# abowman6/CBET_RayTracing_3D

Measured on AMD Instinct MI355X. Metric: ray-steps/sec, OMEGA 60-beam 256^3 sweep, higher is better.
Workload: dtype f64

## Files before the change

cbet_raytracing_3d_amd/api.py:

```python
import ctypes as C
import os

import numpy as np

_PKG = os.path.dirname(os.path.abspath(__file__))
LIB_PATH = os.environ.get("CBET_LIB_PATH") or os.path.join(_PKG, "lib", "libcbet_mi355x.so")
DATA_DIR = os.path.join(_PKG, "data")

OK, EINVAL, EHIP, ENOMEM, ENODEVICE, ECOMM = 0, -1, -2, -3, -4, -5
NPHASE = 2001
KERNEL_DEFAULT, KERNEL_GLOBAL_ATOMICS, KERNEL_LDS_COMBINE, KERNEL_LDS_WINDOW = 0, 1, 2, 3


class CbetError(RuntimeError):
    def __init__(self, code, msg):
        super().__init__("cbet error %d: %s" % (code, msg))
        self.code = code


class Params(C.Structure):
    _fields_ = [
        ("nx", C.c_int), ("ny", C.c_int), ("nz", C.c_int),
        ("xmin", C.c_double), ("xmax", C.c_double),
        ("ymin", C.c_double), ("ymax", C.c_double),
# ... 101 lines not shown
    return hist


EXPORTS = [
    "cbet_last_error", "cbet_version", "cbet_params_default", "cbet_derive",
    "cbet_live_ray_list", "cbet_omega60_beam_norm", "cbet_host_power_table", "cbet_host_beam_trig", "cbet_read_profile",
    "cbet_safeGPUAlloc", "cbet_moveToAndFromGPU", "cbet_gpuFree",
    "cbet_context_create", "cbet_context_destroy", "cbet_context_counters", "cbet_context_tables", "cbet_context_set_launch_list",
    "cbet_launch_ray_XYZ", "cbet_tabulate_plasma", "cbet_trace_nodes", "cbet_prepare_step_records", "cbet_ray_tracing",
    "cbet_write_text", "cbet_edep_average", "cbet_edep_average_device", "cbet_node_coordinates", "cbet_write_npy",
    "cbet_debug_bounds_violations",
    "cbet_gain_params_default", "cbet_gain_constants", "cbet_trace_cbet", "cbet_gain_field",
    "cbet_cbet_workspace_bytes", "cbet_cbet_solve", "cbet_gain_field_slab", "cbet_gain_field_packed",
    "cbet_cbet_slab_workspace_bytes", "cbet_cbet_slab_workspace_bytes_parts", "cbet_pack_segments", "cbet_unpack_segments",
    "cbet_context_list_length", "cbet_cbet_workspace_gain", "cbet_trace_exits", "cbet_exit_tally", "cbet_farfield",
    "cbet_sph_modes_device", "cbet_sph_modes", "cbet_prepare_plasma", "cbet_context_step_records",
]

_lib = None


def lib():
    global _lib
    if _lib is not None:
        return _lib
    import torch
    if not os.path.exists(LIB_PATH):
        raise ImportError(
            "%s is missing: build it with `python -m cbet_raytracing_3d_amd.build` "
            "(hipcc --offload-arch=gfx950).  There is no CPU fallback." % LIB_PATH)
    L = C.CDLL(LIB_PATH)
# ... 8 lines not shown
    L.cbet_host_beam_trig.argtypes = [dp, C.c_int, dp]
    L.cbet_read_profile.argtypes = [C.c_char_p, C.c_int, dp, dp]
    L.cbet_safeGPUAlloc.argtypes = [C.POINTER(vp), C.c_size_t, C.c_int]
    L.cbet_moveToAndFromGPU.argtypes = [vp, vp, C.c_size_t, C.c_int]
    L.cbet_gpuFree.argtypes = [vp, C.c_int]
    L.cbet_context_create.argtypes = [C.POINTER(vp), C.POINTER(Params), C.c_int]
    L.cbet_context_destroy.argtypes = [vp]
    L.cbet_context_counters.argtypes = [vp, vp, C.POINTER(Counters), C.c_int]
    L.cbet_context_set_launch_list.argtypes = [vp, ip, C.c_long]
    L.cbet_context_tables.argtypes = [vp, C.POINTER(vp), C.POINTER(vp)]
    L.cbet_launch_ray_XYZ.argtypes = [C.c_int, C.c_uint, vp, vp, vp, vp, vp, vp, vp, vp,
                                      C.c_double, C.c_double, C.c_double, C.POINTER(Params), vp, vp]
    L.cbet_tabulate_plasma.argtypes = [vp, C.POINTER(Params), vp, vp, vp, vp]
    L.cbet_prepare_step_records.argtypes = [vp, C.POINTER(Params), vp, vp, C.c_double, C.c_double, C.c_double, vp]
    L.cbet_prepare_plasma.argtypes = [vp, C.POINTER(Params), vp, vp, vp, C.c_double, C.c_double, C.c_double, vp]
    L.cbet_context_step_records.argtypes = [vp, C.POINTER(vp), C.POINTER(C.c_ulonglong)]
    L.cbet_trace_nodes.argtypes = [C.c_int, C.c_uint, vp, vp, vp, vp, vp, vp, vp,
                                   C.c_double, C.c_double, C.c_double, C.POINTER(Params), vp, vp]
    L.cbet_ray_tracing.argtypes = [dp, dp, dp, dp, C.POINTER(Params), dp, ip, C.c_int, dp,
                                   C.POINTER(Counters)]
    L.cbet_debug_bounds_violations.argtypes = [C.POINTER(C.c_ulonglong), C.c_int, vp]
    L.cbet_write_text.argtypes = [dp, C.c_int, C.c_int, C.c_int, C.c_char_p]
    L.cbet_write_text.restype = C.c_longlong
    L.cbet_edep_average.argtypes = [dp, dp, C.c_int, C.c_int, C.c_int]
    L.cbet_edep_average_device.argtypes = [vp, vp, C.c_int, C.c_int, C.c_int, vp]
    L.cbet_node_coordinates.argtypes = [C.POINTER(Params), dp, dp, dp]
    L.cbet_write_npy.argtypes = [dp, C.c_int, C.POINTER(C.c_long), C.c_char_p]
    L.cbet_write_npy.restype = C.c_longlong
    L.cbet_gain_params_default.argtypes = [C.POINTER(GainParams)]
    L.cbet_gain_constants.argtypes = [C.POINTER(Params), C.POINTER(GainParams), dp, dp, dp]
# ... 197 lines not shown
def tabulate_plasma(ctx, params, te_data_g, r_data_g, ne_data_g, stream=None):
    _check(lib().cbet_tabulate_plasma(ctx.handle, C.byref(params), _addr(te_data_g),
                                      _addr(r_data_g), _addr(ne_data_g), _addr(stream)))


def prepare_step_records(ctx, params, ne3d, kappa3d, xconst, yconst, zconst, stream=None):
    _check(lib().cbet_prepare_step_records(ctx.handle, C.byref(params), _addr(ne3d), _addr(kappa3d), xconst, yconst,
                                           zconst, _addr(stream)))


def prepare_plasma(ctx, params, te_data_g, r_data_g, ne_data_g, xconst, yconst, zconst, stream=None):
    _check(lib().cbet_prepare_plasma(ctx.handle, C.byref(params), _addr(te_data_g), _addr(r_data_g), _addr(ne_data_g),
                                     xconst, yconst, zconst, _addr(stream)))


def trace_nodes(b, nindices, ne3d, kappa3d, edep, bbeam_norm, beam_norm, pow_r, phase_r, xconst,
                yconst, zconst, params, ctx, stream=None):
    _check(lib().cbet_trace_nodes(
        b, nindices, _addr(ne3d), _addr(kappa3d), _addr(edep), _addr(bbeam_norm), _addr(beam_norm),
        _addr(pow_r), _addr(phase_r), xconst, yconst, zconst, C.byref(params), ctx.handle,
        _addr(stream)))


def default_gain_params(**overrides):
    g = GainParams()
    _check(lib().cbet_gain_params_default(C.byref(g)))
    for k, v in overrides.items():
        setattr(g, k, v)
    return g

# ... 180 lines not shown
```

cbet_raytracing_3d_amd/csrc/cbet_abi.cpp:

```cpp
#include <hip/hip_runtime_api.h>

#include <algorithm>
#include <cmath>
#include <cstdarg>
#include <cstdio>
#include <cstdlib>
#include <cstring>
#include <map>
#include <mutex>
#include <vector>

#include "cbet_device.h"
#include "cbet_mi355x.h"
#include "cbet_omega_beams.h"

namespace cbet {

thread_local char g_err[512] = "";

int fail(int code, const char *fmt, ...)
{
    va_list ap;
    va_start(ap, fmt);
    vsnprintf(g_err, sizeof g_err, fmt, ap);
// ... 196 lines not shown

}

using namespace cbet;

struct cbet_context {
    int gpu = -1;
    cbet_params p{};
    cbet_derived d{};
    double *ne3d = nullptr, *kap3d = nullptr;
    StepRecord *steprec = nullptr;
    unsigned long long tables_version = 0, rec_version = ~0ull;
    unsigned long long rec_builds = 0;
    const double *rec_ne3d = nullptr, *rec_kap3d = nullptr;
    double rec_const[3] = {0, 0, 0};
    double *xlaunch = nullptr, *ylaunch = nullptr;
    double *bounds = nullptr;
    int *live = nullptr;
    int nlive = 0;
    unsigned long long *counters = nullptr;
};

extern "C" {

const char *cbet_last_error(void) { return g_err; }
const char *cbet_version(void) { return "cbet-mi355x 0.1 (gfx950, hip)"; }

int cbet_params_default(cbet_params *p, int n)
{
    if (!p) return fail(CBET_EINVAL, "params is NULL");
// ... 260 lines not shown
{
    if (!out) return fail(CBET_EINVAL, "out is NULL");
    hipError_t e = audit_violations(out, reset != 0, (hipStream_t)stream);
    if (e == hipErrorNotSupported) return fail(CBET_EINVAL, "not a bounds-audit build (compile with -DCBET_DEBUG_BOUNDS)");
    if (e != hipSuccess) return fail(CBET_EHIP, "audit_violations: %s", hipGetErrorString(e));
    return CBET_OK;
}

int cbet_context_list_length(const cbet_context *ctx, long *length)
{
    if (!ctx || !length) return fail(CBET_EINVAL, "NULL context/length");
    *length = ctx->nlive;
    return CBET_OK;
}

int cbet_context_tables(cbet_context *ctx, double **ne3d, double **kappa3d)
{
    if (!ctx) return fail(CBET_EINVAL, "NULL context");
    if (ne3d) *ne3d = ctx->ne3d;
    if (kappa3d) *kappa3d = ctx->kap3d;
    ++ctx->tables_version;
    return CBET_OK;
}

int cbet_context_step_records(const cbet_context *ctx, const void **records, unsigned long long *builds)
{
    if (!ctx) return fail(CBET_EINVAL, "NULL context");
    if (records) *records = ctx->steprec;
    if (builds) *builds = ctx->rec_builds;
    return CBET_OK;
}

static int check_geometry(const cbet_context *ctx, const cbet_params *p)
// ... 5 lines not shown
        p->max_threads != q.max_threads || p->threads_per_block != q.threads_per_block ||
        p->courant_mult != q.courant_mult || p->patch_order != q.patch_order || p->rim_merge != q.rim_merge)
        return fail(CBET_EINVAL, "launch parameters do not match the geometry the context was created for");
    return CBET_OK;
}

int cbet_tabulate_plasma(cbet_context *ctx, const cbet_params *p, const double *te_data_g,
                         const double *r_data_g, const double *ne_data_g, void *stream)
{
    if (!ctx) return fail(CBET_EINVAL, "NULL context");
    if (int rc = validate(p)) return rc;
    if (int rc = check_geometry(ctx, p)) return rc;
    if (!te_data_g || !r_data_g || !ne_data_g) return fail(CBET_EINVAL, "NULL profile pointer");
    DeviceGuard guard;
    CBET_HIP(hipSetDevice(ctx->gpu));
    TabulateArgs t{};
    t.nx = p->nx; t.ny = p->ny; t.nz = p->nz; t.nprofile = p->nprofile;
    t.xmin = p->xmin; t.ymin = p->ymin; t.zmin = p->zmin;
    t.dx = ctx->d.dx; t.dy = ctx->d.dy; t.dz = ctx->d.dz; t.dt = ctx->d.dt;
    t.ncrit = ctx->d.ncrit;
    t.r = r_data_g; t.ne = ne_data_g; t.te = te_data_g;
    t.ne3d = ctx->ne3d; t.kap3d = ctx->kap3d;
    CBET_HIP(launch_tabulate(t, (hipStream_t)stream));
    ++ctx->tables_version;
    return CBET_OK;
}

static int step_records(cbet_context *ctx, const cbet_params *p, const double *ne3d, const double *kappa3d,
                        double xconst, double yconst, double zconst, void *stream, bool force)
{
    const bool own = !ne3d && !kappa3d;
    const double *ne = ne3d ? ne3d : ctx->ne3d, *kap = kappa3d ? kappa3d : ctx->kap3d;
    if (!force && own && ctx->rec_version == ctx->tables_version && ctx->rec_ne3d == ne && ctx->rec_kap3d == kap &&
        ctx->rec_const[0] == xconst && ctx->rec_const[1] == yconst && ctx->rec_const[2] == zconst)
        return CBET_OK;
    StepTableArgs t{};
    t.nx = p->nx; t.ny = p->ny; t.nz = p->nz;
    t.xconst = xconst; t.yconst = yconst; t.zconst = zconst;
    t.ne3d = ne; t.kap3d = kap; t.rec = ctx->steprec;
    CBET_HIP(launch_step_table(t, (hipStream_t)stream));
    ++ctx->rec_builds;
    ctx->rec_version = own ? ctx->tables_version : ~0ull;
    ctx->rec_ne3d = ne; ctx->rec_kap3d = kap;
    ctx->rec_const[0] = xconst; ctx->rec_const[1] = yconst; ctx->rec_const[2] = zconst;
    return CBET_OK;
}

int cbet_prepare_step_records(cbet_context *ctx, const cbet_params *p, const double *ne3d, const double *kappa3d,
                              double xconst, double yconst, double zconst, void *stream)
{
    if (!ctx) return fail(CBET_EINVAL, "NULL context");
    if (int rc = validate(p)) return rc;
    if (int rc = check_geometry(ctx, p)) return rc;
    DeviceGuard guard;
    CBET_HIP(hipSetDevice(ctx->gpu));
    return step_records(ctx, p, ne3d, kappa3d, xconst, yconst, zconst, stream, true);
}

int cbet_prepare_plasma(cbet_context *ctx, const cbet_params *p, const double *te_data_g, const double *r_data_g,
                        const double *ne_data_g, double xconst, double yconst, double zconst, void *stream)
{
    if (!ctx) return fail(CBET_EINVAL, "NULL context");
    if (int rc = validate(p)) return rc;
    if (int rc = check_geometry(ctx, p)) return rc;
    if (!te_data_g || !r_data_g || !ne_data_g) return fail(CBET_EINVAL, "NULL profile pointer");
    if (plasma_records_lds(p->nprofile) > 65536) {
        if (int rc = cbet_tabulate_plasma(ctx, p, te_data_g, r_data_g, ne_data_g, stream)) return rc;
        return cbet_prepare_step_records(ctx, p, nullptr, nullptr, xconst, yconst, zconst, stream);
    }
    DeviceGuard guard;
    CBET_HIP(hipSetDevice(ctx->gpu));
    PlasmaRecordsArgs a{};
    TabulateArgs &t = a.t;
    t.nx = p->nx; t.ny = p->ny; t.nz = p->nz; t.nprofile = p->nprofile;
    t.xmin = p->xmin; t.ymin = p->ymin; t.zmin = p->zmin;
    t.dx = ctx->d.dx; t.dy = ctx->d.dy; t.dz = ctx->d.dz; t.dt = ctx->d.dt;
    t.ncrit = ctx->d.ncrit;
    t.r = r_data_g; t.ne = ne_data_g; t.te = te_data_g;
    t.ne3d = ctx->ne3d; t.kap3d = ctx->kap3d;
    a.xconst = xconst; a.yconst = yconst; a.zconst = zconst;
    a.rec = ctx->steprec;
    CBET_HIP(launch_plasma_records(a, (hipStream_t)stream));
    ++ctx->tables_version;
    ++ctx->rec_builds;
    ctx->rec_version = ctx->tables_version;
    ctx->rec_ne3d = ctx->ne3d; ctx->rec_kap3d = ctx->kap3d;
    ctx->rec_const[0] = xconst; ctx->rec_const[1] = yconst; ctx->rec_const[2] = zconst;
    return CBET_OK;
}

struct CbetHooks {
    const double *gain = nullptr;
    int quantity = 0;
    double *beam_gain = nullptr;
    double max_exponent = 0.0;
    bool exits = false;
};

static int trace_impl(int b, unsigned nindices, const double *ne3d, const double *kappa3d,
                      double *edep, const double *bbeam_norm, const double *beam_norm,
                      const double *pow_r, const double *phase_r, double xconst, double yconst,
                      double zconst, const cbet_params *p, cbet_context *ctx, void *stream,
                      const CbetHooks &hooks)
// ... 41 lines not shown
    a.xconst = xconst; a.yconst = yconst; a.zconst = zconst;
    a.nt = d.nt; a.absorption = p->absorption;
    a.rpz = p->rays_per_zone; a.zones = d.zones_spanned; a.nrays_x = d.nrays_x;
    a.z_launch = kFocal - d.dz / 2;
    a.uray_mult = d.uray_mult; a.omega = d.omega; a.ncrit = d.ncrit;
    a.xlaunch = ctx->xlaunch; a.ylaunch = ctx->ylaunch;
    a.live = ctx->live; a.nlive = ctx->nlive;
    a.beam_lo = beam_lo; a.nbeams_local = beam_hi - beam_lo;
    a.bundles_per_beam = (ctx->nlive + kWave - 1) / kWave;
    a.total_bundles = (long)a.nbeams_local * a.bundles_per_beam;
    {
        const long K = p->shard_count > 1 ? p->shard_count : 1, r = p->shard_count > 1 ? p->shard_index : 0;
        a.first_item = (r * a.total_bundles) / K;
        a.item_count = ((r + 1) * a.total_bundles) / K - a.first_item;
    }
    a.ne3d = ne3d ? ne3d : ctx->ne3d;
    a.kap3d = kappa3d ? kappa3d : ctx->kap3d;
    a.beam_norm = beam_norm; a.bbeam_norm = bbeam_norm; a.pow_r = pow_r; a.phase_r = phase_r;
    a.edep = edep;
    a.sYh = p->edep_zpitch > 0 ? p->edep_zpitch : p->nz + 2;
    a.sXh = (p->ny + 2) * a.sYh;
    if (p->edep_zpitch > 0 && (p->per_beam_grids || cbet_hooks))
        return fail(CBET_EINVAL, "edep_zpitch applies to the plain path's single deposit grid (no per-beam grids, no CBET hooks)");
    a.grid_stride = (p->per_beam_grids || hooks.quantity != 0) ? d.edep_size : 0;
    if (hooks.exits) a.grid_stride = (long)kExitDoubles * ctx->nlive;
    const int gb_n = p->grid_beams > 0 ? p->grid_beams : p->nbeams, gb_0 = p->grid_beams > 0 ? p->grid_beam0 : 0;
    if ((a.grid_stride != 0 || hooks.gain) && (beam_lo < gb_0 || beam_hi > gb_0 + gb_n))
        return fail(CBET_EINVAL, "beams [%d,%d) are not all inside the beam-resolved arrays' range [%d,%d)", beam_lo, beam_hi,
                    gb_0, gb_0 + gb_n);
    a.grid_beam0 = gb_0;
    a.comp_stride = (long)gb_n * d.edep_size;
    a.counters = ctx->counters;
    a.stats = p->window_stats != 0;
    a.gain = hooks.gain; a.hsize = d.edep_size; a.quantity = hooks.quantity;
    a.max_exponent = hooks.max_exponent; a.beam_gain = hooks.beam_gain;
    DeviceGuard guard;
    CBET_HIP(hipSetDevice(ctx->gpu));
    if (variant == CBET_KERNEL_LDS_WINDOW) {
        if (int rc = step_records(ctx, p, ne3d, kappa3d, xconst, yconst, zconst, stream, false)) return rc;
        a.steprec = ctx->steprec;
    }
    CBET_HIP(launch_trace(a, hooks.exits ? kTraceExits : variant, p->force_wide_index != 0, (hipStream_t)stream));
    return CBET_OK;
}

int cbet_trace_nodes(int b, unsigned nindices, const double *ne3d, const double *kappa3d,
                     double *edep, const double *bbeam_norm, const double *beam_norm,
                     const double *pow_r, const double *phase_r, double xconst, double yconst,
                     double zconst, const cbet_params *p, cbet_context *ctx, void *stream)
{
    return trace_impl(b, nindices, ne3d, kappa3d, edep, bbeam_norm, beam_norm, pow_r, phase_r, xconst, yconst,
                      zconst, p, ctx, stream, CbetHooks{});
}

static std::mutex g_ctx_mu;
// ... 18 lines not shown
    g_default_ctx[dev] = ctx;
    *out = ctx;
    return CBET_OK;
}

int cbet_launch_ray_XYZ(int b, unsigned nindices, double *te_data_g, double *r_data_g,
                        double *ne_data_g, double *edep, double *bbeam_norm, double *beam_norm,
                        double *pow_r, double *phase_r, double xconst, double yconst,
                        double zconst, const cbet_params *p, cbet_context *ctx, void *stream)
{
    if (int rc = validate(p)) return rc;
    if (!ctx) {
        if (int rc = default_context(p, &ctx)) return rc;
    }
    const bool records = p->kernel_variant == CBET_KERNEL_DEFAULT || p->kernel_variant == CBET_KERNEL_LDS_WINDOW;
    if (int rc = records ? cbet_prepare_plasma(ctx, p, te_data_g, r_data_g, ne_data_g, xconst, yconst, zconst, stream)
                         : cbet_tabulate_plasma(ctx, p, te_data_g, r_data_g, ne_data_g, stream)) return rc;
    return cbet_trace_nodes(b, nindices, nullptr, nullptr, edep, bbeam_norm, beam_norm, pow_r, phase_r,
                            xconst, yconst, zconst, p, ctx, stream);
}

int cbet_edep_average_device(const double *edep, double *edepavg, int nx, int ny, int nz, void *stream)
{
    if (!edep || !edepavg || nx < 1 || ny < 1 || nz < 1) return fail(CBET_EINVAL, "cbet_edep_average_device: bad array");
    if ((long)(nx + 2) * (ny + 2) * (nz + 2) >= (1L << 31)) return fail(CBET_EINVAL, "cbet_edep_average_device: grid too large");
    CBET_HIP(launch_edep_average(edep, edepavg, nx, ny, nz, (hipStream_t)stream));
    return CBET_OK;
}

int cbet_pack_segments(const double *src, long beam_stride, int hy, int hz, const int *segments, long nseg, double *out,
                       void *stream)
// ... 142 lines not shown
    a.dx = d.dx; a.dy = d.dy; a.dz = d.dz; a.dt = d.dt;
    a.ncrit = d.ncrit; a.k0 = d.omega / kC;
    a.cs = cs; a.gain_const = gc; a.iaw = g->iaw;
    a.mach_r0 = g->mach_r0; a.mach_0 = g->mach_0; a.mach_r1 = g->mach_r1; a.mach_1 = g->mach_1;
    a.relax = g->relax;
    a.fields = fields; a.ne3d = ne3d ? ne3d : ctx->ne3d; a.gain = gain; a.scratch = scratch; a.change = change;
    a.hx_lo = hx_lo; a.hx_hi = hx_hi;
    a.consume = (consume && scratch) ? 1 : 0;
    a.frozen = g->directions_frozen ? 1 : 0;
    const long plane = (long)(p->ny + 2) * (p->nz + 2);
    a.store0 = packed ? (long)hx_lo * plane : 0;
    a.bstride = packed ? (long)(hx_hi - hx_lo) * plane : d.edep_size;
    if (hx_hi == hx_lo) return CBET_OK;
    DeviceGuard guard;
    CBET_HIP(hipSetDevice(ctx->gpu));
    CBET_HIP(launch_gain_field(a, (hipStream_t)stream));
    return CBET_OK;
}

size_t cbet_cbet_workspace_bytes(const cbet_params *p)
{
    if (!p || validate(p) != CBET_OK) return 0;
    const size_t hsize = (size_t)(p->nx + 2) * (p->ny + 2) * (p->nz + 2);
    return (5 * (size_t)p->nbeams * hsize + 2 + CBET_MAX_CBET_BEAMS) * sizeof(double);
}

int cbet_cbet_solve(double *te_data_g, double *r_data_g, double *ne_data_g, double *edep,
                    double *bbeam_norm, double *beam_norm, double *pow_r, double *phase_r,
                    const cbet_params *p, const cbet_gain_params *g, void *workspace,
                    cbet_context *ctx, void *stream, cbet_cbet_report *report)
// ... 139 lines not shown
```

cbet_raytracing_3d_amd/csrc/cbet_device.h:

```cpp
#ifndef CBET_DEVICE_H_
#define CBET_DEVICE_H_

#include <hip/hip_runtime_api.h>

#include "cbet_mi355x.h"

namespace cbet {

constexpr double kC = 29979245800.0;
constexpr double kE0 = 8.85418782e-12;
constexpr double kMe = 9.10938356e-31;
constexpr double kEc = 1.60217662e-19;
constexpr double kLambda = 1.053e-4 / 3.0;
constexpr double kSigma = 0.0375;
constexpr double kIntensity = 1.0e14;
constexpr double kFocal = 0.1;
constexpr double kBeamMin = -450.0e-4;
constexpr double kBeamMax = 450.0e-4;

constexpr unsigned kEmptyTag = 0xFFFFFFFFu;
constexpr int kWave = 64;

enum CounterSlot { kCntSteps = 0, kCntRays = 1, kCntGlobalAtomics = 2, kCntEvictions = 3, kCntWaveSteps = 4,
                   kCntWaveStepsMiss = 5, kCntWaveStepsWide = 6, kCntSlabsRetired = 7, kCntSlots = 8 };
// ... 32 lines not shown
    double fx_hi, fy_hi, fz_hi;
    const double *bounds;
    double tol_x, tol_y, tol_z;
    double xconst, yconst, zconst;
    int nt, absorption;
    int rpz, zones, nrays_x;
    double z_launch;
    double uray_mult, omega, ncrit;
    const double *xlaunch, *ylaunch;
    const int *live;
    int nlive;
    int beam_lo, nbeams_local, bundles_per_beam;
    long total_bundles;
    long first_item, item_count;
    const double *ne3d, *kap3d;
    const StepRecord *steprec;
    const double *beam_norm, *bbeam_norm, *pow_r, *phase_r;
    double *edep;
    int sYh, sXh;
    long grid_stride;
    unsigned long long *counters;
    int stats;
    unsigned long long *audit_count;
    const double *audit_lo, *audit_hi;
    unsigned long long audit_nodes, audit_hsize;
    int grid_beam0;
    const double *gain;
    long hsize;
    int quantity;
    long comp_stride;
// ... 9 lines not shown
    double mach_r0, mach_0, mach_r1, mach_1;
    double relax;
    double *fields;
    const double *ne3d;
    double *gain;
    double *scratch;
    double *change;
    int hx_lo, hx_hi;
    int consume;
    int frozen;
    long store0, bstride;
};

hipError_t launch_tabulate(const TabulateArgs &a, hipStream_t stream);
hipError_t launch_step_table(const StepTableArgs &a, hipStream_t stream);
hipError_t launch_plasma_records(const PlasmaRecordsArgs &a, hipStream_t stream);
size_t plasma_records_lds(int nprofile);
hipError_t audit_violations(unsigned long long *out, bool reset, hipStream_t stream);
hipError_t launch_trace(const TraceArgs &a, int variant, bool force_idx64, hipStream_t stream);
hipError_t launch_trace_window(const TraceArgs &a, bool force_idx64, hipStream_t stream);
constexpr int kTraceExits = 100;
constexpr int kExitDoubles = 10;
hipError_t launch_trace_exit(const TraceArgs &a, bool force_idx64, hipStream_t stream);
hipError_t launch_exit_tally(const cbet_ray_exit *exits, long L, int nbeams, double *tally, hipStream_t stream);
hipError_t launch_farfield(const cbet_ray_exit *exits, long n, int ntheta, int nphi, double *hist, hipStream_t stream);
hipError_t launch_gain_field(const GainArgs &a, hipStream_t stream);
hipError_t launch_pack_segments(const double *src, long beam_stride, int hy, int hz, const int *seg, long nseg, double *out,
                                hipStream_t stream);
hipError_t launch_unpack_segments(double *dst, long beam_stride, int hy, int hz, const int *seg, long nseg, const double *in,
                                  hipStream_t stream);
hipError_t launch_edep_average(const double *edep, double *out, int nx, int ny, int nz, hipStream_t stream);
// ... 19 lines not shown
```

cbet_raytracing_3d_amd/csrc/cbet_kernels.hip:

```cpp
#include <hip/hip_runtime.h>

#include "cbet_trace_common.h"

namespace cbet {
namespace {

__device__ __forceinline__ void interp_table2(const double *y1, const double *y2, const double *x, const double xp,
                                              int n, double &o1, double &o2)
{
    const bool ascending = x[0] <= x[n - 1];
    if (ascending ? (xp <= x[0]) : (xp >= x[0])) { o1 = y1[0]; o2 = y2[0]; return; }
    if (ascending ? (xp >= x[n - 1]) : (xp <= x[n - 1])) { o1 = y1[n - 1]; o2 = y2[n - 1]; return; }
    unsigned lo = 0, hi = n - 1, mid = (lo + hi) >> 1;
    while (lo < hi - 1) {
        const bool go_low = ascending ? (x[mid] >= xp) : !(x[mid] <= xp);
        if (go_low) hi = mid; else lo = mid;
        mid = (lo + hi) >> 1;
    }
    const double dx = x[mid + 1] - x[mid], t = xp - x[mid];
    o1 = y1[mid] + (y1[mid + 1] - y1[mid]) / dx * t;
    o2 = y2[mid] + (y2[mid + 1] - y2[mid]) / dx * t;
}

__device__ __forceinline__ void node_plasma(const TabulateArgs &a, const double *s_r, const double *s_ne, const double *s_te,
// ... 46 lines not shown
        const long oym = (j == 0) ? 0 : ((j == a.ny - 1) ? -2 * sY : -sY), oyp = (j == 0) ? 2 * sY : ((j == a.ny - 1) ? 0 : sY);
        const long ozm = (k == 0) ? 0 : ((k == a.nz - 1) ? -2 : -1), ozp = (k == 0) ? 2 : ((k == a.nz - 1) ? 0 : 1);
        StepRecord r;
        r.kx = a.xconst * (a.ne3d[idx + oxp] - a.ne3d[idx + oxm]);
        r.ky = a.yconst * (a.ne3d[idx + oyp] - a.ne3d[idx + oym]);
        r.kz = a.zconst * (a.ne3d[idx + ozp] - a.ne3d[idx + ozm]);
        r.kap = a.kap3d[idx];
        a.rec[idx] = r;
    }
}

constexpr int kPrTY = 8, kPrTZ = 64, kPrXC = 16, kPrThreads = 256;
constexpr int kPrPZ = kPrTZ + 2;
constexpr int kPrPlane = (kPrTY + 2) * kPrPZ;
constexpr int kPrTile = kPrTY * kPrTZ;
constexpr int kPrItems = kPrTile + 2 * kPrTZ + 2 * kPrTY;

__global__ void __launch_bounds__(kPrThreads) k_plasma_records(const PlasmaRecordsArgs a)
{
    extern __shared__ double s_prof[];
    const TabulateArgs &t = a.t;
    double *s_r = s_prof, *s_ne = s_prof + t.nprofile, *s_te = s_prof + 2 * t.nprofile;
    double *s_ring = s_prof + 3 * t.nprofile;
    double *s_kap = s_ring + 3 * kPrPlane;
    const int tid = threadIdx.x;
    for (int i = tid; i < t.nprofile; i += kPrThreads) {
        s_r[i] = t.r[i];
        s_ne[i] = t.ne[i];
        s_te[i] = t.te[i];
    }
    __syncthreads();
    const int nx = t.nx, ny = t.ny, nz = t.nz;
    const int k0 = max(0, min((int)blockIdx.x * kPrTZ, nz - kPrTZ));
    const int j0 = max(0, min((int)blockIdx.y * kPrTY, ny - kPrTY));
    const int x0 = (int)blockIdx.z * kPrXC, x1 = min(x0 + kPrXC, nx);
    const int pa = x0 == 0 ? 0 : min(x0 - 1, nx - 3);
    const int pb = x1 == nx ? nx : max(x1 + 1, 3);

    auto emit = [&](int i, int xl, int xh) {
        const double *lo = s_ring + (xl % 3) * kPrPlane, *hi = s_ring + (xh % 3) * kPrPlane, *mid = s_ring + (i % 3) * kPrPlane;
        const double *kap = s_kap + (i % 3) * kPrTile;
        for (int q = tid; q < 2 * kPrTile; q += kPrThreads) {
            const int n = q >> 1, jr = n / kPrTZ, kr = n % kPrTZ;
            const int j = j0 + jr, k = k0 + kr;
            if (j >= ny || k >= nz) continue;
            const int c = (jr + 1) * kPrPZ + kr + 1;
            double v0, v1;
            if ((q & 1) == 0) {
                const int ym = (j == 0) ? 0 : ((j == ny - 1) ? -2 : -1), yp = (j == 0) ? 2 : ((j == ny - 1) ? 0 : 1);
                v0 = a.xconst * (hi[c] - lo[c]);
                v1 = a.yconst * (mid[c + yp * kPrPZ] - mid[c + ym * kPrPZ]);
            } else {
                const int zm = (k == 0) ? 0 : ((k == nz - 1) ? -2 : -1), zp = (k == 0) ? 2 : ((k == nz - 1) ? 0 : 1);
                v0 = a.zconst * (mid[c + zp] - mid[c + zm]);
                v1 = kap[n];
            }
            const long idx = ((long)i * ny + j) * nz + k;
            reinterpret_cast<double2 *>(a.rec + idx)[q & 1] = make_double2(v0, v1);
        }
    };

    for (int p = pa; p < pb; ++p) {
        const bool own_plane = p >= x0 && p < x1;
        double *ring = s_ring + (p % 3) * kPrPlane;
        for (int n = tid; n < (own_plane ? kPrItems : kPrTile); n += kPrThreads) {
            int jj, kk;
            if (n < kPrTile) {
                jj = 1 + n / kPrTZ; kk = 1 + n % kPrTZ;
            } else if (n < kPrTile + 2 * kPrTZ) {
                const int h = n - kPrTile;
                jj = h < kPrTZ ? 0 : kPrTY + 1; kk = 1 + h % kPrTZ;
            } else {
                const int h = n - kPrTile - 2 * kPrTZ;
                kk = h < kPrTY ? 0 : kPrTZ + 1; jj = 1 + h % kPrTY;
            }
            const int j = j0 + jj - 1, k = k0 + kk - 1;
            if (j < 0 || j >= ny || k < 0 || k >= nz) continue;
            double ed, kap;
            if (own_plane && n < kPrTile) {
                node_plasma(t, s_r, s_ne, s_te, p, j, k, ed, kap);
                s_kap[(p % 3) * kPrTile + n] = kap;
                const long idx = ((long)p * ny + j) * nz + k;
                t.ne3d[idx] = ed;
                t.kap3d[idx] = kap;
            } else {
                node_plasma(t, s_r, s_ne, s_te, p, j, k, ed, kap);
            }
            ring[jj * kPrPZ + kk] = ed;
        }
        __syncthreads();
        if (p == 2 && x0 == 0) emit(0, 0, 2);
        if (p - 1 >= 1 && p - 1 >= x0 && p - 1 < x1) emit(p - 1, p - 2, p);
        if (p == nx - 1 && x1 == nx) emit(nx - 1, nx - 3, nx - 1);
        __syncthreads();
    }
}

template <int WL>
struct LdsWindow {
    static constexpr int W = 1 << WL;
    static constexpr int NSLOT = W * W * W;
    double *val;
    unsigned *tag;
    const TraceArgs *args;

    __device__ __forceinline__ unsigned slot(int i, int j, int k) const
    {
        return (unsigned)((((i & (W - 1)) << WL) | (j & (W - 1))) << WL | (k & (W - 1)));
    }
// ... 203 lines not shown
    hipLaunchKernelGGL(k_tabulate, dim3((unsigned)blocks), dim3(256), lds, stream, a);
    return hipGetLastError();
}

hipError_t launch_step_table(const StepTableArgs &a, hipStream_t stream)
{
    const long total = (long)a.nx * a.ny * a.nz;
    long blocks = (total + 255) / 256;
    if (blocks > 256 * 16) blocks = 256 * 16;
    hipLaunchKernelGGL(k_step_table, dim3((unsigned)blocks), dim3(256), 0, stream, a);
    return hipGetLastError();
}

size_t plasma_records_lds(int nprofile)
{
    return sizeof(double) * (3 * (size_t)nprofile + 3 * (size_t)kPrPlane + 3 * (size_t)kPrTile);
}

hipError_t launch_plasma_records(const PlasmaRecordsArgs &a, hipStream_t stream)
{
    const dim3 grid((unsigned)((a.t.nz + kPrTZ - 1) / kPrTZ), (unsigned)((a.t.ny + kPrTY - 1) / kPrTY),
                    (unsigned)((a.t.nx + kPrXC - 1) / kPrXC));
    hipLaunchKernelGGL(k_plasma_records, grid, dim3(kPrThreads), plasma_records_lds(a.t.nprofile), stream, a);
    return hipGetLastError();
}

hipError_t audit_violations(unsigned long long *out, bool reset, hipStream_t stream)
{
#ifdef CBET_DEBUG_BOUNDS
    hipError_t e = hipStreamSynchronize(stream);
    if (e != hipSuccess) return e;
    e = hipMemcpyFromSymbol(out, HIP_SYMBOL(g_audit_violations), sizeof *out);
    if (e == hipSuccess && reset) {
        const unsigned long long zero = 0;
        e = hipMemcpyToSymbol(HIP_SYMBOL(g_audit_violations), &zero, sizeof zero);
    }
    return e;
#else
// ... 32 lines not shown
```

cbet_raytracing_3d_amd/csrc/cbet_trace_common.h:

```cpp
#ifndef CBET_TRACE_COMMON_H_
#define CBET_TRACE_COMMON_H_

#include <hip/hip_runtime.h>

#include "cbet_device.h"
#include "cbet_relocate.h"

namespace cbet {

__device__ __forceinline__ double interp_table(const double *y, const double *x, const double xp, int n)
{
    unsigned lo, hi, mid;
    if (x[0] <= x[n - 1]) {
        if (xp <= x[0]) return y[0];
        if (xp >= x[n - 1]) return y[n - 1];
        lo = 0;
        hi = n - 1;
        mid = (lo + hi) >> 1;
        while (lo < hi - 1) {
            if (x[mid] >= xp) hi = mid; else lo = mid;
            mid = (lo + hi) >> 1;
        }
    } else {
        if (xp >= x[0]) return y[0];
// ... 63 lines not shown
    const double keep2 = x0;
    x0 = x0 * c2 - y0 * s2;
    y0 = y0 * c2 + keep2 * s2;

    s.px = x0;
    s.py = y0;
    s.pz = z0;
    s.uray = a.uray_mult * interp_table(a.pow_r, a.phase_r, ref, CBET_NPHASE);
    s.ustop = 0.05 * s.uray;
    if (!(ref <= kBeamMax)) return false;

    s.ci = first_node_within(s.px, a.xmin, a.dx, a.tol_x, a.nx);
    s.cj = first_node_within(s.py, a.ymin, a.dy, a.tol_y, a.ny);
    s.ck = first_node_within(s.pz, a.zmin, a.dz, a.tol_z, a.nz);

    const double ne0 = a.ne3d[((long)s.ci * a.ny + s.cj) * a.nz + s.ck];
    const double w = sqrt((a.omega * a.omega - ne0 * 1e6 * (kEc * kEc) / ((double)kMe * kE0)) / (kC * kC));
    double vx = -1 * bnx, vy = -1 * bny, vz = -1 * bnz;
    const double knorm = sqrt(vx * vx + vy * vy + vz * vz);
    s.vx = (kC * kC) * ((vx / knorm) * w) / a.omega;
    s.vy = (kC * kC) * ((vy / knorm) * w) / a.omega;
    s.vz = (kC * kC) * ((vz / knorm) * w) / a.omega;
    return true;
}

#ifdef CBET_DEBUG_BOUNDS
__device__ __forceinline__ bool audit_fail(const TraceArgs &a)
{
    atomicAdd(a.audit_count, 1ull);
    return true;
}
// ... 118 lines not shown
```

cbet_raytracing_3d_amd/tracer.py:

```python
import os

import numpy as np
import torch

from . import api


class RayTracer:

    def __init__(self, params, r_profile, ne_profile, te_profile, beam_norm=None, device=None):
        if not torch.cuda.is_available():
            raise RuntimeError("RayTracer needs a HIP device (no CPU fallback)")
        self.device = torch.device("cuda", torch.cuda.current_device()) if device is None \
            else torch.device(device)
        self.gpu = self.device.index if self.device.index is not None else torch.cuda.current_device()
        self.params = params.copy()
        self.derived = api.derive(self.params)
        if beam_norm is None:
            beam_norm = api.omega60_beam_norm()[: self.params.nbeams]
        beam_norm = np.ascontiguousarray(beam_norm, dtype=np.float64).reshape(-1, 3)
        if beam_norm.shape[0] != self.params.nbeams:
            raise ValueError("beam_norm has %d rows, params.nbeams=%d" % (beam_norm.shape[0], self.params.nbeams))
        phase_r, pow_r = api.host_power_table()
        bbeam = api.host_beam_trig(beam_norm)
# ... 269 lines not shown
        self.launch_p = p.copy(beam_lo=0, beam_hi=p.nbeams, shard_index=si, shard_count=sc,
                               edep_zpitch=zp if pad_rows else 0)
        self.passes = 0

    def run_pass(self, timed=False):
        tr, d, b = self.tr, self.tr.derived, self.passes % 2
        self.passes += 1
        with torch.cuda.stream(self.s_prep[b]):
            sp = self.s_prep[b].cuda_stream
            if self.ev_trace[b] is not None:
                self.s_prep[b].wait_event(self.ev_trace[b])
            if self.work[b] is not None:
                self.work[b].wait()
                self.work[b] = None
            self.grids[b].zero_()
            api.prepare_plasma(self.ctx[b], self.launch_p, tr.d_te, tr.d_r, tr.d_ne, d.xconst, d.yconst, d.zconst, sp)
            self.ev_prep[b].record()
        with torch.cuda.stream(self.s_trace[b]):
            st = self.s_trace[b].cuda_stream
            self.s_trace[b].wait_event(self.ev_prep[b])
            if timed:
                e0, e1 = torch.cuda.Event(enable_timing=True), torch.cuda.Event(enable_timing=True)
                e0.record()
            api.trace_nodes(0, d.nindices, None, None, self.grids[b], tr.d_bbeam_norm, tr.d_beam_norm, tr.d_pow_r,
                            tr.d_phase_r, d.xconst, d.yconst, d.zconst, self.launch_p, self.ctx[b], st)
            if timed:
                e1.record()
                self.kernel_events.append((e0, e1))
            consumed, self.ev_consumed[b] = self.ev_consumed[b], None
            if consumed is not None:
                self.s_trace[b].wait_event(consumed)
# ... 755 lines not shown
```

include/cbet_mi355x.h:

```cpp
#ifndef CBET_MI355X_H_
#define CBET_MI355X_H_

#include <stddef.h>

#ifdef __cplusplus
extern "C" {
#endif

#define CBET_OK 0
#define CBET_EINVAL (-1)
#define CBET_EHIP (-2)
#define CBET_ENOMEM (-3)
#define CBET_ENODEVICE (-4)
#define CBET_ECOMM (-5)

#define CBET_NPHASE 2001
#define CBET_MAX_CBET_BEAMS 64

#define CBET_KERNEL_DEFAULT 0
#define CBET_KERNEL_GLOBAL_ATOMICS 1
#define CBET_KERNEL_LDS_COMBINE 2
#define CBET_KERNEL_LDS_WINDOW 3

#define CBET_BEAMS_BY_GPU (-1)
// ... 84 lines not shown
                        double *pow_r, double *phase_r, double xconst, double yconst,
                        double zconst, const cbet_params *p, cbet_context *ctx, void *stream);

int cbet_tabulate_plasma(cbet_context *ctx, const cbet_params *p, const double *te_data_g,
                         const double *r_data_g, const double *ne_data_g, void *stream);
int cbet_trace_nodes(int b, unsigned nindices, const double *ne3d, const double *kappa3d,
                     double *edep, const double *bbeam_norm, const double *beam_norm,
                     const double *pow_r, const double *phase_r, double xconst, double yconst,
                     double zconst, const cbet_params *p, cbet_context *ctx, void *stream);
int cbet_prepare_step_records(cbet_context *ctx, const cbet_params *p, const double *ne3d,
                              const double *kappa3d, double xconst, double yconst, double zconst,
                              void *stream);
int cbet_prepare_plasma(cbet_context *ctx, const cbet_params *p, const double *te_data_g,
                        const double *r_data_g, const double *ne_data_g, double xconst, double yconst,
                        double zconst, void *stream);

int cbet_ray_tracing(const double *te_profile, const double *r_profile, const double *ne_profile,
                     double *edep, const cbet_params *p, const double *beam_norm, const int *gpus,
                     int ngpu, double *timers, cbet_counters *counters);

long long cbet_write_text(const double *edep, int d0, int d1, int d2, const char *path);
int cbet_edep_average(const double *edep, double *edepavg, int nx, int ny, int nz);
int cbet_edep_average_device(const double *edep, double *edepavg, int nx, int ny, int nz, void *stream);
int cbet_node_coordinates(const cbet_params *p, double *x, double *y, double *z);
long long cbet_write_npy(const double *data, int ndim, const long *shape, const char *path);

typedef struct cbet_gain_params {
    double z_ion;
    double te_ev, ti_ev;
    double mi_over_me;
// ... 104 lines not shown
```

Baseline: 167.2 billion.

## Defer ne3d/kappa3d table writes when only step records are needed

Adds a records-only prepare path that builds the step records without writing the dense ne3d and kappa3d tables, and marks the tables as pending so they are built lazily if another consumer asks for them. The trace launch computes the initial density by interpolating the radial profile when the tables are absent. The plasma-records kernel is also restructured so each lane pair owns fixed tile nodes and keeps kappa in registers instead of an LDS ring, and halo nodes get one lane each. This cuts global writes and LDS use in the prepare step, at the cost of more complex pending-state bookkeeping and a stream-dependent lazy build.

```diff
diff --git a/cbet_raytracing_3d_amd/api.py b/cbet_raytracing_3d_amd/api.py
--- a/cbet_raytracing_3d_amd/api.py
+++ b/cbet_raytracing_3d_amd/api.py
@@ -139,7 +139,7 @@
     "cbet_cbet_workspace_bytes", "cbet_cbet_solve", "cbet_gain_field_slab", "cbet_gain_field_packed",
     "cbet_cbet_slab_workspace_bytes", "cbet_cbet_slab_workspace_bytes_parts", "cbet_pack_segments", "cbet_unpack_segments",
     "cbet_context_list_length", "cbet_cbet_workspace_gain", "cbet_trace_exits", "cbet_exit_tally", "cbet_farfield",
-    "cbet_sph_modes_device", "cbet_sph_modes", "cbet_prepare_plasma", "cbet_context_step_records",
+    "cbet_sph_modes_device", "cbet_sph_modes", "cbet_prepare_plasma", "cbet_prepare_records", "cbet_context_step_records",
 ]
 
 _lib = None
@@ -178,6 +178,7 @@
     L.cbet_tabulate_plasma.argtypes = [vp, C.POINTER(Params), vp, vp, vp, vp]
     L.cbet_prepare_step_records.argtypes = [vp, C.POINTER(Params), vp, vp, C.c_double, C.c_double, C.c_double, vp]
     L.cbet_prepare_plasma.argtypes = [vp, C.POINTER(Params), vp, vp, vp, C.c_double, C.c_double, C.c_double, vp]
+    L.cbet_prepare_records.argtypes = [vp, C.POINTER(Params), vp, vp, vp, C.c_double, C.c_double, C.c_double, vp]
     L.cbet_context_step_records.argtypes = [vp, C.POINTER(vp), C.POINTER(C.c_ulonglong)]
     L.cbet_trace_nodes.argtypes = [C.c_int, C.c_uint, vp, vp, vp, vp, vp, vp, vp,
                                    C.c_double, C.c_double, C.c_double, C.POINTER(Params), vp, vp]
@@ -405,6 +406,11 @@
                                      xconst, yconst, zconst, _addr(stream)))
 
 
+def prepare_records(ctx, params, te_data_g, r_data_g, ne_data_g, xconst, yconst, zconst, stream=None):
+    _check(lib().cbet_prepare_records(ctx.handle, C.byref(params), _addr(te_data_g), _addr(r_data_g), _addr(ne_data_g),
+                                      xconst, yconst, zconst, _addr(stream)))
+
+
 def trace_nodes(b, nindices, ne3d, kappa3d, edep, bbeam_norm, beam_norm, pow_r, phase_r, xconst,
                 yconst, zconst, params, ctx, stream=None):
     _check(lib().cbet_trace_nodes(
diff --git a/cbet_raytracing_3d_amd/csrc/cbet_abi.cpp b/cbet_raytracing_3d_amd/csrc/cbet_abi.cpp
--- a/cbet_raytracing_3d_amd/csrc/cbet_abi.cpp
+++ b/cbet_raytracing_3d_amd/csrc/cbet_abi.cpp
@@ -234,6 +234,9 @@
     unsigned long long rec_builds = 0;
     const double *rec_ne3d = nullptr, *rec_kap3d = nullptr;
     double rec_const[3] = {0, 0, 0};
+    bool tables_pending = false;
+    const double *pend_te = nullptr, *pend_r = nullptr, *pend_ne = nullptr;
+    void *pend_stream = nullptr;
     double *xlaunch = nullptr, *ylaunch = nullptr;
     double *bounds = nullptr;
     int *live = nullptr;
@@ -524,9 +527,37 @@
     return CBET_OK;
 }
 
+static TabulateArgs tabulate_args(const cbet_context *ctx, const cbet_params *p, const double *te, const double *r,
+                                  const double *ne)
+{
+    TabulateArgs t{};
+    t.nx = p->nx; t.ny = p->ny; t.nz = p->nz; t.nprofile = p->nprofile;
+    t.xmin = p->xmin; t.ymin = p->ymin; t.zmin = p->zmin;
+    t.dx = ctx->d.dx; t.dy = ctx->d.dy; t.dz = ctx->d.dz; t.dt = ctx->d.dt;
+    t.ncrit = ctx->d.ncrit;
+    t.r = r; t.ne = ne; t.te = te;
+    t.ne3d = ctx->ne3d; t.kap3d = ctx->kap3d;
+    return t;
+}
+
+static int ensure_tables(cbet_context *ctx, void *stream)
+{
+    if (!ctx->tables_pending) return CBET_OK;
+    CBET_HIP(launch_tabulate(tabulate_args(ctx, &ctx->p, ctx->pend_te, ctx->pend_r, ctx->pend_ne), (hipStream_t)stream));
+    ctx->tables_pending = false;
+    return CBET_OK;
+}
+
 int cbet_context_tables(cbet_context *ctx, double **ne3d, double **kappa3d)
 {
     if (!ctx) return fail(CBET_EINVAL, "NULL context");
+    if (ctx->tables_pending) {
+        DeviceGuard guard;
+        CBET_HIP(hipSetDevice(ctx->gpu));
+        void *stream = ctx->pend_stream;
+        if (int rc = ensure_tables(ctx, stream)) return rc;
+        CBET_HIP(hipStreamSynchronize((hipStream_t)stream));
+    }
     if (ne3d) *ne3d = ctx->ne3d;
     if (kappa3d) *kappa3d = ctx->kap3d;
     ++ctx->tables_version;
@@ -562,15 +593,9 @@
     if (!te_data_g || !r_data_g || !ne_data_g) return fail(CBET_EINVAL, "NULL profile pointer");
     DeviceGuard guard;
     CBET_HIP(hipSetDevice(ctx->gpu));
-    TabulateArgs t{};
-    t.nx = p->nx; t.ny = p->ny; t.nz = p->nz; t.nprofile = p->nprofile;
-    t.xmin = p->xmin; t.ymin = p->ymin; t.zmin = p->zmin;
-    t.dx = ctx->d.dx; t.dy = ctx->d.dy; t.dz = ctx->d.dz; t.dt = ctx->d.dt;
-    t.ncrit = ctx->d.ncrit;
-    t.r = r_data_g; t.ne = ne_data_g; t.te = te_data_g;
-    t.ne3d = ctx->ne3d; t.kap3d = ctx->kap3d;
-    CBET_HIP(launch_tabulate(t, (hipStream_t)stream));
+    CBET_HIP(launch_tabulate(tabulate_args(ctx, p, te_data_g, r_data_g, ne_data_g), (hipStream_t)stream));
     ++ctx->tables_version;
+    ctx->tables_pending = false;
     return CBET_OK;
 }
 
@@ -582,6 +607,8 @@
     if (!force && own && ctx->rec_version == ctx->tables_version && ctx->rec_ne3d == ne && ctx->rec_kap3d == kap &&
         ctx->rec_const[0] == xconst && ctx->rec_const[1] == yconst && ctx->rec_const[2] == zconst)
         return CBET_OK;
+    if (!ne3d || !kappa3d)
+        if (int rc = ensure_tables(ctx, stream)) return rc;
     StepTableArgs t{};
     t.nx = p->nx; t.ny = p->ny; t.nz = p->nz;
     t.xconst = xconst; t.yconst = yconst; t.zconst = zconst;
@@ -605,8 +632,8 @@
     return step_records(ctx, p, ne3d, kappa3d, xconst, yconst, zconst, stream, true);
 }
 
-int cbet_prepare_plasma(cbet_context *ctx, const cbet_params *p, const double *te_data_g, const double *r_data_g,
-                        const double *ne_data_g, double xconst, double yconst, double zconst, void *stream)
+static int prepare_plasma(cbet_context *ctx, const cbet_params *p, const double *te_data_g, const double *r_data_g,
+                          const double *ne_data_g, double xconst, double yconst, double zconst, void *stream, bool tables)
 {
     if (!ctx) return fail(CBET_EINVAL, "NULL context");
     if (int rc = validate(p)) return rc;
@@ -619,22 +646,30 @@
     DeviceGuard guard;
     CBET_HIP(hipSetDevice(ctx->gpu));
     PlasmaRecordsArgs a{};
-    TabulateArgs &t = a.t;
-    t.nx = p->nx; t.ny = p->ny; t.nz = p->nz; t.nprofile = p->nprofile;
-    t.xmin = p->xmin; t.ymin = p->ymin; t.zmin = p->zmin;
-    t.dx = ctx->d.dx; t.dy = ctx->d.dy; t.dz = ctx->d.dz; t.dt = ctx->d.dt;
-    t.ncrit = ctx->d.ncrit;
-    t.r = r_data_g; t.ne = ne_data_g; t.te = te_data_g;
-    t.ne3d = ctx->ne3d; t.kap3d = ctx->kap3d;
+    a.t = tabulate_args(ctx, p, te_data_g, r_data_g, ne_data_g);
     a.xconst = xconst; a.yconst = yconst; a.zconst = zconst;
     a.rec = ctx->steprec;
-    CBET_HIP(launch_plasma_records(a, (hipStream_t)stream));
+    CBET_HIP(launch_plasma_records(a, tables, (hipStream_t)stream));
     ++ctx->tables_version;
     ++ctx->rec_builds;
     ctx->rec_version = ctx->tables_version;
     ctx->rec_ne3d = ctx->ne3d; ctx->rec_kap3d = ctx->kap3d;
     ctx->rec_const[0] = xconst; ctx->rec_const[1] = yconst; ctx->rec_const[2] = zconst;
-    return CBET_OK;
+    ctx->tables_pending = !tables;
+    ctx->pend_te = te_data_g; ctx->pend_r = r_data_g; ctx->pend_ne = ne_data_g; ctx->pend_stream = stream;
+    return CBET_OK;
+}
+
+int cbet_prepare_plasma(cbet_context *ctx, const cbet_params *p, const double *te_data_g, const double *r_data_g,
+                        const double *ne_data_g, double xconst, double yconst, double zconst, void *stream)
+{
+    return prepare_plasma(ctx, p, te_data_g, r_data_g, ne_data_g, xconst, yconst, zconst, stream, true);
+}
+
+int cbet_prepare_records(cbet_context *ctx, const cbet_params *p, const double *te_data_g, const double *r_data_g,
+                         const double *ne_data_g, double xconst, double yconst, double zconst, void *stream)
+{
+    return prepare_plasma(ctx, p, te_data_g, r_data_g, ne_data_g, xconst, yconst, zconst, stream, false);
 }
 
 struct CbetHooks {
@@ -706,8 +741,6 @@
         a.first_item = (r * a.total_bundles) / K;
         a.item_count = ((r + 1) * a.total_bundles) / K - a.first_item;
     }
-    a.ne3d = ne3d ? ne3d : ctx->ne3d;
-    a.kap3d = kappa3d ? kappa3d : ctx->kap3d;
     a.beam_norm = beam_norm; a.bbeam_norm = bbeam_norm; a.pow_r = pow_r; a.phase_r = phase_r;
     a.edep = edep;
     a.sYh = p->edep_zpitch > 0 ? p->edep_zpitch : p->nz + 2;
@@ -731,6 +764,14 @@
     if (variant == CBET_KERNEL_LDS_WINDOW) {
         if (int rc = step_records(ctx, p, ne3d, kappa3d, xconst, yconst, zconst, stream, false)) return rc;
         a.steprec = ctx->steprec;
+    } else if (!ne3d || !kappa3d) {
+        if (int rc = ensure_tables(ctx, stream)) return rc;
+    }
+    a.ne3d = ne3d ? ne3d : ctx->ne3d;
+    a.kap3d = kappa3d ? kappa3d : ctx->kap3d;
+    if (!ne3d && ctx->tables_pending) {
+        a.ne3d = nullptr;
+        a.prof_r = ctx->pend_r; a.prof_ne = ctx->pend_ne; a.nprofile = p->nprofile;
     }
     CBET_HIP(launch_trace(a, hooks.exits ? kTraceExits : variant, p->force_wide_index != 0, (hipStream_t)stream));
     return CBET_OK;
@@ -779,7 +820,7 @@
         if (int rc = default_context(p, &ctx)) return rc;
     }
     const bool records = p->kernel_variant == CBET_KERNEL_DEFAULT || p->kernel_variant == CBET_KERNEL_LDS_WINDOW;
-    if (int rc = records ? cbet_prepare_plasma(ctx, p, te_data_g, r_data_g, ne_data_g, xconst, yconst, zconst, stream)
+    if (int rc = records ? cbet_prepare_records(ctx, p, te_data_g, r_data_g, ne_data_g, xconst, yconst, zconst, stream)
                          : cbet_tabulate_plasma(ctx, p, te_data_g, r_data_g, ne_data_g, stream)) return rc;
     return cbet_trace_nodes(b, nindices, nullptr, nullptr, edep, bbeam_norm, beam_norm, pow_r, phase_r,
                             xconst, yconst, zconst, p, ctx, stream);
@@ -952,6 +993,8 @@
     if (hx_hi == hx_lo) return CBET_OK;
     DeviceGuard guard;
     CBET_HIP(hipSetDevice(ctx->gpu));
+    if (!ne3d)
+        if (int rc = ensure_tables(ctx, stream)) return rc;
     CBET_HIP(launch_gain_field(a, (hipStream_t)stream));
     return CBET_OK;
 }
diff --git a/cbet_raytracing_3d_amd/csrc/cbet_device.h b/cbet_raytracing_3d_amd/csrc/cbet_device.h
--- a/cbet_raytracing_3d_amd/csrc/cbet_device.h
+++ b/cbet_raytracing_3d_amd/csrc/cbet_device.h
@@ -70,6 +70,8 @@
     long total_bundles;
     long first_item, item_count;
     const double *ne3d, *kap3d;
+    const double *prof_r, *prof_ne;
+    int nprofile;
     const StepRecord *steprec;
     const double *beam_norm, *bbeam_norm, *pow_r, *phase_r;
     double *edep;
@@ -109,7 +111,7 @@
 
 hipError_t launch_tabulate(const TabulateArgs &a, hipStream_t stream);
 hipError_t launch_step_table(const StepTableArgs &a, hipStream_t stream);
-hipError_t launch_plasma_records(const PlasmaRecordsArgs &a, hipStream_t stream);
+hipError_t launch_plasma_records(const PlasmaRecordsArgs &a, bool tables, hipStream_t stream);
 size_t plasma_records_lds(int nprofile);
 hipError_t audit_violations(unsigned long long *out, bool reset, hipStream_t stream);
 hipError_t launch_trace(const TraceArgs &a, int variant, bool force_idx64, hipStream_t stream);
diff --git a/cbet_raytracing_3d_amd/csrc/cbet_kernels.hip b/cbet_raytracing_3d_amd/csrc/cbet_kernels.hip
--- a/cbet_raytracing_3d_amd/csrc/cbet_kernels.hip
+++ b/cbet_raytracing_3d_amd/csrc/cbet_kernels.hip
@@ -84,15 +84,19 @@
 constexpr int kPrPZ = kPrTZ + 2;
 constexpr int kPrPlane = (kPrTY + 2) * kPrPZ;
 constexpr int kPrTile = kPrTY * kPrTZ;
-constexpr int kPrItems = kPrTile + 2 * kPrTZ + 2 * kPrTY;
-
+constexpr int kPrHalo = 2 * kPrTZ + 2 * kPrTY;
+constexpr int kPrPairs = kPrThreads / 2;
+constexpr int kPrOwn = kPrTile / kPrThreads;
+static_assert(kPrTile == 4 * kPrPairs && kPrOwn == 2, "a lane pair owns four tile nodes, each lane two of them");
+static_assert(kPrHalo <= kPrThreads, "one halo node per lane");
+
+template <bool TABLES>
 __global__ void __launch_bounds__(kPrThreads) k_plasma_records(const PlasmaRecordsArgs a)
 {
     extern __shared__ double s_prof[];
     const TabulateArgs &t = a.t;
     double *s_r = s_prof, *s_ne = s_prof + t.nprofile, *s_te = s_prof + 2 * t.nprofile;
     double *s_ring = s_prof + 3 * t.nprofile;
-    double *s_kap = s_ring + 3 * kPrPlane;
     const int tid = threadIdx.x;
     for (int i = tid; i < t.nprofile; i += kPrThreads) {
         s_r[i] = t.r[i];
@@ -106,63 +110,82 @@
     const int x0 = (int)blockIdx.z * kPrXC, x1 = min(x0 + kPrXC, nx);
     const int pa = x0 == 0 ? 0 : min(x0 - 1, nx - 3);
     const int pb = x1 == nx ? nx : max(x1 + 1, 3);
-
-    auto emit = [&](int i, int xl, int xh) {
+    const int pair = tid >> 1, parity = tid & 1;
+
+    auto emit = [&](int i, int xl, int xh, const double (&kap)[kPrOwn]) {
         const double *lo = s_ring + (xl % 3) * kPrPlane, *hi = s_ring + (xh % 3) * kPrPlane, *mid = s_ring + (i % 3) * kPrPlane;
-        const double *kap = s_kap + (i % 3) * kPrTile;
-        for (int q = tid; q < 2 * kPrTile; q += kPrThreads) {
-            const int n = q >> 1, jr = n / kPrTZ, kr = n % kPrTZ;
+#pragma nounroll
+        for (int m = 0; m < 4; ++m) {
+            const int n = pair + kPrPairs * m, jr = n / kPrTZ, kr = n % kPrTZ;
             const int j = j0 + jr, k = k0 + kr;
             if (j >= ny || k >= nz) continue;
             const int c = (jr + 1) * kPrPZ + kr + 1;
+            const bool mine = (m & 1) == parity;
             double v0, v1;
-            if ((q & 1) == 0) {
+            if (!mine) {
                 const int ym = (j == 0) ? 0 : ((j == ny - 1) ? -2 : -1), yp = (j == 0) ? 2 : ((j == ny - 1) ? 0 : 1);
                 v0 = a.xconst * (hi[c] - lo[c]);
                 v1 = a.yconst * (mid[c + yp * kPrPZ] - mid[c + ym * kPrPZ]);
             } else {
                 const int zm = (k == 0) ? 0 : ((k == nz - 1) ? -2 : -1), zp = (k == 0) ? 2 : ((k == nz - 1) ? 0 : 1);
                 v0 = a.zconst * (mid[c + zp] - mid[c + zm]);
-                v1 = kap[n];
+                v1 = (m & 2) ? kap[1] : kap[0];
             }
             const long idx = ((long)i * ny + j) * nz + k;
-            reinterpret_cast<double2 *>(a.rec + idx)[q & 1] = make_double2(v0, v1);
+            reinterpret_cast<double2 *>(a.rec + idx)[mine ? 1 : 0] = make_double2(v0, v1);
         }
     };
 
+    double kap_now[kPrOwn] = {}, kap_prev[kPrOwn] = {}, kap_first[kPrOwn] = {};
     for (int p = pa; p < pb; ++p) {
         const bool own_plane = p >= x0 && p < x1;
         double *ring = s_ring + (p % 3) * kPrPlane;
-        for (int n = tid; n < (own_plane ? kPrItems : kPrTile); n += kPrThreads) {
-            int jj, kk;
-            if (n < kPrTile) {
-                jj = 1 + n / kPrTZ; kk = 1 + n % kPrTZ;
-            } else if (n < kPrTile + 2 * kPrTZ) {
-                const int h = n - kPrTile;
-                jj = h < kPrTZ ? 0 : kPrTY + 1; kk = 1 + h % kPrTZ;
-            } else {
-                const int h = n - kPrTile - 2 * kPrTZ;
-                kk = h < kPrTY ? 0 : kPrTZ + 1; jj = 1 + h % kPrTY;
-            }
-            const int j = j0 + jj - 1, k = k0 + kk - 1;
-            if (j < 0 || j >= ny || k < 0 || k >= nz) continue;
+#pragma nounroll
+        for (int s = 0; s < kPrOwn; ++s) {
+            const int n = pair + kPrPairs * (parity + 2 * s), jr = n / kPrTZ, kr = n % kPrTZ;
+            const int j = j0 + jr, k = k0 + kr;
+            if (j >= ny || k >= nz) continue;
             double ed, kap;
-            if (own_plane && n < kPrTile) {
+            if (own_plane) {
                 node_plasma(t, s_r, s_ne, s_te, p, j, k, ed, kap);
-                s_kap[(p % 3) * kPrTile + n] = kap;
-                const long idx = ((long)p * ny + j) * nz + k;
-                t.ne3d[idx] = ed;
-                t.kap3d[idx] = kap;
+                if (s == 0) kap_now[0] = kap; else kap_now[1] = kap;
+                if (TABLES) {
+                    const long idx = ((long)p * ny + j) * nz + k;
+                    t.ne3d[idx] = ed;
+                    t.kap3d[idx] = kap;
+                }
             } else {
                 node_plasma(t, s_r, s_ne, s_te, p, j, k, ed, kap);
             }
-            ring[jj * kPrPZ + kk] = ed;
+            ring[(jr + 1) * kPrPZ + kr + 1] = ed;
+        }
+        if (own_plane && tid < kPrHalo) {
+            int jj, kk;
+            if (tid < 2 * kPrTZ) {
+                jj = tid < kPrTZ ? 0 : kPrTY + 1; kk = 1 + tid % kPrTZ;
+            } else {
+                const int h = tid - 2 * kPrTZ;
+                kk = h < kPrTY ? 0 : kPrTZ + 1; jj = 1 + h % kPrTY;
+            }
+            const int j = j0 + jj - 1, k = k0 + kk - 1;
+            if (j >= 0 && j < ny && k >= 0 && k < nz) {
+                double ed, kap;
+                node_plasma(t, s_r, s_ne, s_te, p, j, k, ed, kap);
+                ring[jj * kPrPZ + kk] = ed;
+            }
         }
         __syncthreads();
-        if (p == 2 && x0 == 0) emit(0, 0, 2);
-        if (p - 1 >= 1 && p - 1 >= x0 && p - 1 < x1) emit(p - 1, p - 2, p);
-        if (p == nx - 1 && x1 == nx) emit(nx - 1, nx - 3, nx - 1);
+        if (p == 2 && x0 == 0) emit(0, 0, 2, kap_first);
+        if (p - 1 >= 1 && p - 1 >= x0 && p - 1 < x1) emit(p - 1, p - 2, p, kap_prev);
+        if (p == nx - 1 && x1 == nx) emit(nx - 1, nx - 3, nx - 1, kap_now);
         __syncthreads();
+        if (own_plane) {
+#pragma unroll
+            for (int s = 0; s < kPrOwn; ++s) {
+                kap_prev[s] = kap_now[s];
+                if (p == 0) kap_first[s] = kap_now[s];
+            }
+        }
     }
 }
 
@@ -396,14 +419,16 @@
 
 size_t plasma_records_lds(int nprofile)
 {
-    return sizeof(double) * (3 * (size_t)nprofile + 3 * (size_t)kPrPlane + 3 * (size_t)kPrTile);
-}
-
-hipError_t launch_plasma_records(const PlasmaRecordsArgs &a, hipStream_t stream)
+    return sizeof(double) * (3 * (size_t)nprofile + 3 * (size_t)kPrPlane);
+}
+
+hipError_t launch_plasma_records(const PlasmaRecordsArgs &a, bool tables, hipStream_t stream)
 {
     const dim3 grid((unsigned)((a.t.nz + kPrTZ - 1) / kPrTZ), (unsigned)((a.t.ny + kPrTY - 1) / kPrTY),
                     (unsigned)((a.t.nx + kPrXC - 1) / kPrXC));
-    hipLaunchKernelGGL(k_plasma_records, grid, dim3(kPrThreads), plasma_records_lds(a.t.nprofile), stream, a);
+    const size_t lds = plasma_records_lds(a.t.nprofile);
+    if (tables) hipLaunchKernelGGL(k_plasma_records<true>, grid, dim3(kPrThreads), lds, stream, a);
+    else hipLaunchKernelGGL(k_plasma_records<false>, grid, dim3(kPrThreads), lds, stream, a);
     return hipGetLastError();
 }
 
diff --git a/cbet_raytracing_3d_amd/csrc/cbet_trace_common.h b/cbet_raytracing_3d_amd/csrc/cbet_trace_common.h
--- a/cbet_raytracing_3d_amd/csrc/cbet_trace_common.h
+++ b/cbet_raytracing_3d_amd/csrc/cbet_trace_common.h
@@ -101,7 +101,13 @@
     s.cj = first_node_within(s.py, a.ymin, a.dy, a.tol_y, a.ny);
     s.ck = first_node_within(s.pz, a.zmin, a.dz, a.tol_z, a.nz);
 
-    const double ne0 = a.ne3d[((long)s.ci * a.ny + s.cj) * a.nz + s.ck];
+    double ne0;
+    if (a.ne3d) {
+        ne0 = a.ne3d[((long)s.ci * a.ny + s.cj) * a.nz + s.ck];
+    } else {
+        const double xc = s.ci * a.dx + a.xmin, yc = s.cj * a.dy + a.ymin, zc = s.ck * a.dz + a.zmin;
+        ne0 = interp_table(a.prof_ne, a.prof_r, sqrt(xc * xc + yc * yc + zc * zc), a.nprofile);
+    }
     const double w = sqrt((a.omega * a.omega - ne0 * 1e6 * (kEc * kEc) / ((double)kMe * kE0)) / (kC * kC));
     double vx = -1 * bnx, vy = -1 * bny, vz = -1 * bnz;
     const double knorm = sqrt(vx * vx + vy * vy + vz * vz);
diff --git a/cbet_raytracing_3d_amd/tracer.py b/cbet_raytracing_3d_amd/tracer.py
--- a/cbet_raytracing_3d_amd/tracer.py
+++ b/cbet_raytracing_3d_amd/tracer.py
@@ -307,7 +307,7 @@
                 self.work[b].wait()
                 self.work[b] = None
             self.grids[b].zero_()
-            api.prepare_plasma(self.ctx[b], self.launch_p, tr.d_te, tr.d_r, tr.d_ne, d.xconst, d.yconst, d.zconst, sp)
+            api.prepare_records(self.ctx[b], self.launch_p, tr.d_te, tr.d_r, tr.d_ne, d.xconst, d.yconst, d.zconst, sp)
             self.ev_prep[b].record()
         with torch.cuda.stream(self.s_trace[b]):
             st = self.s_trace[b].cuda_stream
diff --git a/include/cbet_mi355x.h b/include/cbet_mi355x.h
--- a/include/cbet_mi355x.h
+++ b/include/cbet_mi355x.h
@@ -122,6 +122,9 @@
 int cbet_prepare_plasma(cbet_context *ctx, const cbet_params *p, const double *te_data_g,
                         const double *r_data_g, const double *ne_data_g, double xconst, double yconst,
                         double zconst, void *stream);
+int cbet_prepare_records(cbet_context *ctx, const cbet_params *p, const double *te_data_g,
+                         const double *r_data_g, const double *ne_data_g, double xconst, double yconst,
+                         double zconst, void *stream);
 
 int cbet_ray_tracing(const double *te_profile, const double *r_profile, const double *ne_profile,
                      double *edep, const cbet_params *p, const double *beam_norm, const int *gpus,
```

Result: no change. 168.2 billion (median of 6 runs) (+0.6%).
